# ctu-vras/depth_correction

Measured on AMD Instinct MI355X. Metric: points/sec through min_eigval_loss fwd+bwd (200k pts, k=10); HBM GB/s vs peak, higher is better.
Workload: dtype f64

## Files before the change

depth_correction_amd/csrc/dc_consistency.hip:

```cpp
#include <type_traits>
#include <atomic>
#include <mutex>
#include <cstdio>
#include <hip/hip_ext.h>
#include "dc_common.h"
#include "dc_device.h"
#include "dc_pointmath.h"
#include "dc_prof.h"
#include "dc_points_dev.h"
#include "../../include/dc_hip.h"

namespace dc {

template <typename T, typename PT, int STRIDE>
__global__ __launch_bounds__(kBlock) void points_fwd_kernel(PointInputs in, int64_t n, QParams qp, PT* __restrict__ x_out,
                                                            T* __restrict__ vps_out, T* __restrict__ dirs_out,
                                                            T* __restrict__ depth_out) {
  __shared__ double s_pose[kLdsScans * 12];
  const int64_t i = (int64_t)blockIdx.x * kBlock + threadIdx.x;
  const int64_t ic = i < n ? i : n - 1;
  ModelParams mp;
  load_model(in, mp);
  T vp_r[3] = {T(0), T(0), T(0)}, dr_r[3];
  if (in.vps) { const T* q = (const T*)in.vps + ic * 3; vp_r[0] = q[0]; vp_r[1] = q[1]; vp_r[2] = q[2]; }
// ... 1643 lines not shown
#pragma unroll
      for (int q = 1; q < NS; ++q) mx = max(mx, pre[q]);
      const bool any_miss = __any((int)(mx == kNoLoc)) != 0;
      int n_have;
      if (any_miss) n_have = gather_fixed<PT, NS, true>(tile, cap, ci, pre, acc);
      else n_have = gather_fixed<PT, NS, false>(tile, cap, ci, pre, acc);
      acc.W = (double)n_have;
      double cm[3], v0[3], c1, c2;
      if constexpr ((VAR & kVarSlimTail) != 0) step_point2<PT, NS>(acc, n_have, !any_miss, in_mask, lp, qp, acc2, cm, v0, &c1, &c2);
      else step_point<PT>(acc, in_mask, lp, qp, acc2, cm, v0, &c1, &c2);
      const double u = Pt<PT>::unit(qp);
      if constexpr ((VAR & kVarF32Sweep) != 0 && std::is_same<PT, q32>::value) {
        float cmf[3], vs[3], vu[3], gwf[P];
#pragma unroll
        for (int a = 0; a < 3; ++a) { cmf[a] = (float)cm[a]; vs[a] = (float)(c1 * v0[a]); vu[a] = (float)v0[a]; }
        const float c2f = (float)c2;
#pragma unroll
        for (int k = 0; k < P; ++k) gwf[k] = 0.0f;
        if (any_miss) {
#pragma unroll
          for (int q = 0; q < NS; ++q) {
            if (q % 4 == 0 && q > 0) __builtin_amdgcn_sched_barrier(0);
            chain_term_f32<P>(tile, cap, pre[q], pre[q] != kNoLoc, ci, cmf, vs, vu, c2f, gwf);
          }
        } else {
#pragma unroll
          for (int q = 0; q < NS; ++q) {
            if (q % 4 == 0 && q > 0) __builtin_amdgcn_sched_barrier(0);
            chain_term_f32<P>(tile, cap, pre[q], true, ci, cmf, vs, vu, c2f, gwf);
          }
        }
#pragma unroll
        for (int k = 0; k < P; ++k) gw[k] = (double)gwf[k] * u;
      } else {
        double mean[3];
        StepRow<PT, P>::mean_of(ci, cm, mean);
        if (any_miss) {
#pragma unroll
          for (int q = 0; q < NS; ++q) chain_term<PT, P>(tile, cap, pre[q], pre[q] != kNoLoc, mean, v0, c1, c2, gw);
        } else {
#pragma unroll
          for (int q = 0; q < NS; ++q) chain_term<PT, P>(tile, cap, pre[q], true, mean, v0, c1, c2, gw);
        }
#pragma unroll
        for (int k = 0; k < P; ++k) gw[k] *= u;
      }
    }
  }
  if (bad) acc2[0] = acc2[1] = __longlong_as_double(0x7ff8000000000000ll);
  step_partials<P, (VAR & kVarDppSums) != 0>(acc2, gw, p_fwd, p_bwd, chained, chained ? ch.n_front : 0);
}

constexpr int kStepQ32Cap = 512;

typedef float float2v __attribute__((ext_vector_type(2)));
template <int P, int CAP>
__device__ __forceinline__ void chain_term_q32(const int4* tile, uint32_t off, bool have, const Pt<q32>::Raw& ci, const float* cmf, const float* vs,
                                               const float* vu, float c2f, float* gw) {
  const char* row = reinterpret_cast<const char*>(tile) + (have ? off : 0u);
  const int4 p0 = *reinterpret_cast<const int4*>(row);
  const int4 p1 = *reinterpret_cast<const int4*>(row + (size_t)CAP * 16);
  const float2v e01 = float2v{(float)(p0.x - ci.v[0]), (float)(p0.y - ci.v[1])} - float2v{cmf[0], cmf[1]};
  const float e0 = e01.x, e1 = e01.y, e2 = (float)(p0.z - ci.v[2]) - cmf[2];
  const float u0 = __int_as_float(p0.w), u1 = __int_as_float(p1.x), u2 = __int_as_float(p1.y);
  const float al = fmaf(vs[2], e2, fmaf(vs[1], e1, vs[0] * e0));
  const float be = fmaf(vu[2], u2, fmaf(vu[1], u1, vu[0] * u0));
  const float ga = fmaf(e2, u2, fmaf(e1, u1, e0 * u0));
  float tj = fmaf(al, be, -(c2f * ga));
  if (!have) tj = 0.0f;
  if constexpr (P == 2) {
    float2v g = float2v{gw[0], gw[1]};
    g = __builtin_elementwise_fma(float2v{tj, tj}, float2v{__int_as_float(p1.z), __int_as_float(p1.w)}, g);
    gw[0] = g.x; gw[1] = g.y;
  } else {
    gw[0] = fmaf(tj, __int_as_float(p1.z), gw[0]);
    if constexpr (P > 1) gw[1] = fmaf(tj, __int_as_float(p1.w), gw[1]);
    if constexpr (P > 2) gw[2] = fmaf(tj, __int_as_float(reinterpret_cast<const int4*>(row + (size_t)CAP * 32)->x), gw[2]);
  }
}

#ifdef DC_BLOCK_TRACE
__device__ unsigned long long* g_block_trace = nullptr;
#define DC_TRACE_BEGIN() const unsigned long long trace_t0 = __builtin_amdgcn_s_memrealtime()
#define DC_TRACE_END() do { if (threadIdx.x == 0 && g_block_trace) { \
    unsigned long long* tr_ = g_block_trace + 4 * (size_t)blockIdx.x; \
    tr_[0] = ((unsigned long long)__builtin_amdgcn_s_getreg((31 << 11) | 20) << 32) | (unsigned)__builtin_amdgcn_s_getreg((31 << 11) | 4); \
    tr_[1] = trace_t0; tr_[2] = __builtin_amdgcn_s_memrealtime(); tr_[3] = 1; } } while (0)
#else
#define DC_TRACE_BEGIN() do {} while (0)
#define DC_TRACE_END() do {} while (0)
#endif

template <int NS, int P, int CAP>
__global__ __launch_bounds__(kBlock, (StepRow<q32, P>::kPieces * CAP * 16 <= 25 * 1024 ? 6 : 4)) void consistency_step_q32_kernel(
    PointBasis pb, BlockTab tab, const int32_t* __restrict__ own_base, const int32_t* __restrict__ centre_idx, int64_t n,
    const uint8_t* __restrict__ mask, LossParams lp, QParams qp, double* __restrict__ p_fwd, double* __restrict__ p_bwd,
    StepChain ch) {
  constexpr int NV = 2 + P, NP2 = NV <= 4 ? 4 : 8;
  constexpr int cap = CAP;
  __shared__ int4 tile[StepRow<q32, P>::kPieces * CAP];
  __shared__ double s_w[DC_MAX_MODEL_TERMS];
  __shared__ double s_front[kWavesPerBlock];
  __shared__ double s_comb[kWavesPerBlock * NP2];
  __shared__ int s_ok[2];
  DC_TRACE_BEGIN();
  const bool chained = ch.ready != nullptr;
  if (chained && (int)blockIdx.x < ch.n_front) { chain_front_block<P>(ch, s_front); return; }
  const int64_t nblocks = (n + kBlock - 1) / kBlock;
  int64_t blk = chain_block_of(ch, chained, nblocks);
  if (blk >= 0 && ch.blk_skip && ch.blk_skip[blk]) blk = -1;
  double acc2[2] = {0.0, 0.0}, gw[P];
#pragma unroll
  for (int k = 0; k < P; ++k) gw[k] = 0.0;
  const int32_t s0 = blk >= 0 ? tab.slot_ptr[blk] : 0;
  bool bad = blk >= 0 && tab.slot_ptr[blk + 1] - s0 != NS;
  if (blk >= 0 && !bad) {
    const int64_t i = blk * kBlock + threadIdx.x;
    const bool live = i < n;
    const bool in_mask = live && (mask ? mask[i] != 0 : true);
    const uint16_t* lrow = tab.loc + (int64_t)s0 * kBlock + threadIdx.x;
    uint32_t pre[NS];
#pragma unroll
    for (int q = 0; q < NS; ++q) pre[q] = (uint32_t)lrow[q * kBlock];
    const int32_t base = tab.blk_ptr[blk], nd = tab.blk_ptr[blk + 1] - base;
    const int32_t own = (own_base && !centre_idx) ? own_base[blk] : -1;
    double wq[P];
    if (chained) {
      typename StepRow<q32, P>::Raw r0, r1;
      const int t0 = threadIdx.x, t1 = threadIdx.x + kBlock;
      if (t0 < nd) r0 = StepRow<q32, P>::fetch(pb, tab.blk_ids[base + t0]);
      if (t1 < nd) r1 = StepRow<q32, P>::fetch(pb, tab.blk_ids[base + t1]);
      chain_weights<P>(ch, pb.w_scale, s_w, s_ok);
      __syncthreads();
      if (!s_ok[0]) bad = true;
#pragma unroll
      for (int k = 0; k < P; ++k) wq[k] = s_w[k];
      if (t0 < nd) StepRow<q32, P>::place(r0, wq, tile, cap, t0);
      if (t1 < nd) StepRow<q32, P>::place(r1, wq, tile, cap, t1);
      for (int t = threadIdx.x + 2 * kBlock; t < nd; t += kBlock) StepRow<q32, P>::stage(pb, wq, tab.blk_ids[base + t], tile, cap, t);
    } else {
      stage_weights(pb, s_w);
      __syncthreads();
#pragma unroll
      for (int k = 0; k < P; ++k) wq[k] = s_w[k];
      for (int t = threadIdx.x; t < nd; t += kBlock) StepRow<q32, P>::stage(pb, wq, tab.blk_ids[base + t], tile, cap, t);
    }
    Pt<q32>::Raw ci;
    if (own < 0) ci = Basis<q32>::template point<P>(pb, wq, live ? (centre_idx ? (int64_t)centre_idx[i] : i) : 0);
    __syncthreads();
    if (own >= 0) ci = staged_point<q32>(tile, cap, own + (live ? (int)threadIdx.x : 0));
    if (live && (!mask || __any((int)in_mask))) {
      CovAcc acc;
      cov_init(acc);
      uint32_t mo = pre[0];
#pragma unroll
      for (int q = 1; q < NS; ++q) mo |= pre[q];
      const bool any_miss = __any((int)(mo & 1u)) != 0;
      int n_have;
      if (any_miss) n_have = gather_fixed<q32, NS, true>(tile, cap, ci, pre, acc);
      else n_have = gather_fixed<q32, NS, false>(tile, cap, ci, pre, acc);
      acc.W = (double)n_have;
      double cm[3], v0[3], c1, c2;
      step_point2<q32, NS>(acc, n_have, !any_miss, in_mask, lp, qp, acc2, cm, v0, &c1, &c2);
      float cmf[3], vs[3], vu[3], gwf[P];
#pragma unroll
      for (int a = 0; a < 3; ++a) { cmf[a] = (float)cm[a]; vs[a] = (float)(c1 * v0[a]); vu[a] = (float)v0[a]; }
      const float c2f = (float)c2;
#pragma unroll
      for (int k = 0; k < P; ++k) gwf[k] = 0.0f;
      if (any_miss) {
#pragma unroll
        for (int q = 0; q < NS; ++q) {
          if (q % 4 == 0 && q > 0) __builtin_amdgcn_sched_barrier(0);
          chain_term_q32<P, CAP>(tile, pre[q], pre[q] != kNoLoc, ci, cmf, vs, vu, c2f, gwf);
        }
      } else {
#pragma unroll
        for (int q = 0; q < NS; ++q) {
          if (q % 4 == 0 && q > 0) __builtin_amdgcn_sched_barrier(0);
          chain_term_q32<P, CAP>(tile, pre[q], true, ci, cmf, vs, vu, c2f, gwf);
        }
      }
      const double u = qp.scale;
#pragma unroll
      for (int k = 0; k < P; ++k) gw[k] = (double)gwf[k] * u;
    }
  }
  if (bad) acc2[0] = acc2[1] = __longlong_as_double(0x7ff8000000000000ll);
  double v[NP2];
  v[0] = acc2[0]; v[1] = acc2[1];
#pragma unroll
  for (int k = 0; k < NP2 - 2; ++k) v[2 + k] = k < P ? gw[k] : 0.0;
  double tot;
  if constexpr (NP2 == 4) tot = wave_sum4_dpp(v);
  else tot = wave_sum_packed<NP2>(v);
  const int lane = threadIdx.x & (kWave - 1), wave = threadIdx.x / kWave;
  int64_t rs = (int64_t)gridDim.x * kWavesPerBlock, row = (int64_t)blockIdx.x * kWavesPerBlock + wave;
  if (chained) {
    if (lane < NP2) s_comb[wave * NP2 + lane] = tot;
    __syncthreads();
    if (wave != 0) return;
    if (lane < NP2) tot = (s_comb[lane] + s_comb[NP2 + lane]) + (s_comb[2 * NP2 + lane] + s_comb[3 * NP2 + lane]);
    rs = (int64_t)gridDim.x - ch.n_front;
    row = (int64_t)blockIdx.x - ch.n_front;
  }
  if (lane < NP2) {
    const int q = packed_value_of_lane<NP2>(lane);
    if (q < 2) p_fwd[q * rs + row] = tot;
    else if (q < NV) p_bwd[(q - 2) * rs + row] = tot;
  }
  DC_TRACE_END();
}

template <typename PT, int P>
__global__ __launch_bounds__(kBlock) void consistency_step_basis_slots_kernel(
    PointBasis pb, BlockTab tab, const int32_t* __restrict__ own_base, int cap, const int32_t* __restrict__ centre_idx, int64_t n,
    const uint8_t* __restrict__ mask, LossParams lp, QParams qp, double* __restrict__ p_fwd, double* __restrict__ p_bwd,
    StepChain ch, int packed) {
  extern __shared__ int4 tile[];
  __shared__ double s_w[DC_MAX_MODEL_TERMS];
  __shared__ int s_ok;
  __shared__ double s_front[kBlock / kWave];
  const bool chained = ch.ready != nullptr;
  if (chained && (int)blockIdx.x < ch.n_front) { chain_front_block<P>(ch, s_front); return; }
  const int64_t nblocks = (n + kBlock - 1) / kBlock;
  int64_t blk = xcd_block_of((int64_t)blockIdx.x - (chained ? ch.n_front : 0), nblocks);
  if (blk >= 0 && ch.blk_skip && ch.blk_skip[blk]) blk = -1;
  double acc2[2] = {0.0, 0.0}, gw[P];
#pragma unroll
  for (int k = 0; k < P; ++k) gw[k] = 0.0;
  const int64_t i = blk * kBlock + threadIdx.x;
  const bool live = blk >= 0 && i < n;
  int32_t nslots = 0, own = -1, base = 0, nd = 0;
  const uint16_t* lrow = tab.loc;
  uint32_t pre[kPreSlots];
  if (blk >= 0) {
    const int32_t s0 = tab.slot_ptr[blk];
    nslots = tab.slot_ptr[blk + 1] - s0;
    lrow = tab.loc + (int64_t)s0 * kBlock + threadIdx.x;
#pragma unroll
    for (int q = 0; q < kPreSlots; ++q) pre[q] = (live && q < nslots) ? (uint32_t)lrow[q * kBlock] : kNoLoc;
    own = (own_base && !centre_idx) ? own_base[blk] : -1;
    base = tab.blk_ptr[blk];
    nd = tab.blk_ptr[blk + 1] - base;
  }
  double wq[P];
  bool timed_out = false;
  typename Pt<PT>::Raw ci;
  if (chained) {
    typename StepRow<PT, P>::Raw r0, r1;
    const int t0 = threadIdx.x, t1 = threadIdx.x + kBlock;
    if (t0 < nd) r0 = StepRow<PT, P>::fetch(pb, tab.blk_ids[base + t0]);
    if (t1 < nd) r1 = StepRow<PT, P>::fetch(pb, tab.blk_ids[base + t1]);
    chain_weights<P>(ch, pb.w_scale, s_w, &s_ok);
    __syncthreads();
    timed_out = !s_ok;
#pragma unroll
    for (int k = 0; k < P; ++k) wq[k] = s_w[k];
    if (t0 < nd) StepRow<PT, P>::place(r0, wq, tile, cap, t0);
    if (t1 < nd) StepRow<PT, P>::place(r1, wq, tile, cap, t1);
    for (int t = threadIdx.x + 2 * kBlock; t < nd; t += kBlock) StepRow<PT, P>::stage(pb, wq, tab.blk_ids[base + t], tile, cap, t);
  } else {
    stage_weights(pb, s_w);
    __syncthreads();
#pragma unroll
    for (int k = 0; k < P; ++k) wq[k] = s_w[k];
    for (int t = threadIdx.x; t < nd; t += kBlock) StepRow<PT, P>::stage(pb, wq, tab.blk_ids[base + t], tile, cap, t);
  }
  if (blk >= 0 && own < 0) ci = Basis<PT>::template point<P>(pb, wq, live ? (centre_idx ? (int64_t)centre_idx[i] : i) : 0);
  __syncthreads();
  if (live) {
    if (own >= 0) ci = staged_point<PT>(tile, cap, own + (int)threadIdx.x);
    CovAcc acc;
    cov_init(acc);
    bool miss = false;
#pragma unroll
    for (int q = 0; q < kPreSlots; ++q) miss |= (q < nslots) && pre[q] == kNoLoc;
    int n_have = 0;
    if (__any((int)miss)) n_have = gather_slots<PT, true>(tile, cap, ci, pre, nslots, acc);
    else n_have = gather_slots<PT, false>(tile, cap, ci, pre, nslots, acc);
    if (nslots > kPreSlots) n_have += gather_tail<PT>(tile, cap, ci, lrow, nslots, packed != 0, acc);
    acc.W = (double)n_have;
    double cm[3], v0[3], c1, c2;
    step_point2<PT, 2>(acc, n_have, false, mask ? mask[i] != 0 : true, lp, qp, acc2, cm, v0, &c1, &c2);
    const double u = Pt<PT>::unit(qp);
    if constexpr (std::is_same<PT, q32>::value) {
      float cmf[3], vs[3], vu[3], gwf[P];
#pragma unroll
      for (int a = 0; a < 3; ++a) { cmf[a] = (float)cm[a]; vs[a] = (float)(c1 * v0[a]); vu[a] = (float)v0[a]; }
      const float c2f = (float)c2;
#pragma unroll
      for (int k = 0; k < P; ++k) gwf[k] = 0.0f;
#pragma unroll
      for (int q = 0; q < kPreSlots; ++q)
// ... 89 lines not shown
    cov_init(acc);
    auto sweep1 = [&](const uint32_t* l, uint32_t* nx, const uint16_t* pn) {
#pragma unroll
      for (int u_ = 0; u_ < kTrip; ++u_) nx[u_] = (uint32_t)pn[u_ * kBlock];
      int4 r[kTrip];
#pragma unroll
      for (int u_ = 0; u_ < kTrip; ++u_) r[u_] = *reinterpret_cast<const int4*>(tb + (l[u_] == kNoLoc ? own_off : l[u_]));
#pragma unroll
      for (int u_ = 0; u_ < kTrip; ++u_)
        cov_add_d(acc, (double)(r[u_].x - ci.v[0]), (double)(r[u_].y - ci.v[1]), (double)(r[u_].z - ci.v[2]));
    };
    {
      uint32_t la[kTrip], lb[kTrip];
#pragma unroll
      for (int u_ = 0; u_ < kTrip; ++u_) la[u_] = first[u_];
      const uint16_t* pn = lrow + kTrip * kBlock;
      for (int q0 = 0; q0 < wmax; q0 += 2 * kTrip) {
        sweep1(la, lb, pn);
        pn += kTrip * kBlock;
        if (q0 + kTrip >= wmax) break;
        sweep1(lb, la, pn);
        pn += kTrip * kBlock;
      }
    }
    acc.W = (double)deg;
    double cm[3], v0[3], c1, c2;
    step_point2<q32, 2>(acc, deg, false, in_mask, lp, qp, acc2, cm, v0, &c1, &c2);
    const double u = Pt<q32>::unit(qp);
    float cmf[3], vs[3], vu[3];
#pragma unroll
    for (int a = 0; a < 3; ++a) { cmf[a] = (float)cm[a]; vs[a] = (float)(c1 * v0[a]); vu[a] = (float)v0[a]; }
    const float c2f = (float)c2;
    auto sweep2 = [&](const uint32_t* l, uint32_t* nx, const uint16_t* pn) {
#pragma unroll
      for (int u_ = 0; u_ < kTrip; ++u_) nx[u_] = (uint32_t)pn[u_ * kBlock];
      float2v g[P];
#pragma unroll
      for (int k = 0; k < P; ++k) g[k] = float2v{0.0f, 0.0f};
#pragma unroll
      for (int u_ = 0; u_ < kTrip; u_ += 2) {
        const bool ha = l[u_] != kNoLoc, hb = l[u_ + 1] != kNoLoc;
        const char* ra = tb + (ha ? l[u_] : own_off);
        const char* rb = tb + (hb ? l[u_ + 1] : own_off);
        const int4 a0 = *reinterpret_cast<const int4*>(ra), a1 = *reinterpret_cast<const int4*>(ra + CAP * 16);
        const int4 b0 = *reinterpret_cast<const int4*>(rb), b1 = *reinterpret_cast<const int4*>(rb + CAP * 16);
        const float2v e0 = float2v{(float)(a0.x - ci.v[0]), (float)(b0.x - ci.v[0])} - float2v{cmf[0], cmf[0]};
        const float2v e1 = float2v{(float)(a0.y - ci.v[1]), (float)(b0.y - ci.v[1])} - float2v{cmf[1], cmf[1]};
        const float2v e2 = float2v{(float)(a0.z - ci.v[2]), (float)(b0.z - ci.v[2])} - float2v{cmf[2], cmf[2]};
        const float2v u0 = float2v{__int_as_float(a0.w), __int_as_float(b0.w)};
        const float2v u1 = float2v{__int_as_float(a1.x), __int_as_float(b1.x)};
        const float2v u2 = float2v{__int_as_float(a1.y), __int_as_float(b1.y)};
        const float2v al = __builtin_elementwise_fma(float2v{vs[2], vs[2]}, e2, __builtin_elementwise_fma(float2v{vs[1], vs[1]}, e1, float2v{vs[0], vs[0]} * e0));
        const float2v be = __builtin_elementwise_fma(float2v{vu[2], vu[2]}, u2, __builtin_elementwise_fma(float2v{vu[1], vu[1]}, u1, float2v{vu[0], vu[0]} * u0));
        const float2v ga = __builtin_elementwise_fma(e2, u2, __builtin_elementwise_fma(e1, u1, e0 * u0));
        float2v tj = __builtin_elementwise_fma(al, be, -(float2v{c2f, c2f} * ga));
        tj = float2v{ha ? tj.x : 0.0f, hb ? tj.y : 0.0f};
        g[0] = __builtin_elementwise_fma(tj, float2v{__int_as_float(a1.z), __int_as_float(b1.z)}, g[0]);
        if constexpr (P > 1) g[1] = __builtin_elementwise_fma(tj, float2v{__int_as_float(a1.w), __int_as_float(b1.w)}, g[1]);
        if constexpr (P > 2)
          g[2] = __builtin_elementwise_fma(tj, float2v{__int_as_float(reinterpret_cast<const int4*>(ra + CAP * 32)->x),
                                                       __int_as_float(reinterpret_cast<const int4*>(rb + CAP * 32)->x)}, g[2]);
      }
#pragma unroll
      for (int k = 0; k < P; ++k) gw[k] += (double)(g[k].x + g[k].y);
    };
    {
      uint32_t la[kTrip], lb[kTrip];
#pragma unroll
      for (int u_ = 0; u_ < kTrip; ++u_) la[u_] = first[u_];
      const uint16_t* pn = lrow + kTrip * kBlock;
      for (int q0 = 0; q0 < wmax; q0 += 2 * kTrip) {
        sweep2(la, lb, pn);
        pn += kTrip * kBlock;
        if (q0 + kTrip >= wmax) break;
        sweep2(lb, la, pn);
        pn += kTrip * kBlock;
      }
    }
#pragma unroll
    for (int k = 0; k < P; ++k) gw[k] *= u;
  }
  if (timed_out) acc2[0] = acc2[1] = __longlong_as_double(0x7ff8000000000000ll);
  step_partials<P, true>(acc2, gw, p_fwd, p_bwd, chained, chained ? ch.n_front : 0);
  DC_TRACE_END();
}

struct PoseTab {
  const int32_t* __restrict__ blk_ptr;
  const int32_t* __restrict__ ids;
  const uint16_t* __restrict__ loc;
  const uint16_t* __restrict__ own_pos;
  const uint16_t* __restrict__ row_seg;
  const uint8_t* __restrict__ row_scan;
};
constexpr int kPoseCap = 512;

template <int K>
__global__ __launch_bounds__(kBlock) void pose_table_kernel(BlockTab tab, const int32_t* __restrict__ own_base,
                                                            const int32_t* __restrict__ scan_id, int64_t n, int n_scans,
                                                            int32_t* __restrict__ ids_out, uint16_t* __restrict__ loc_out,
                                                            uint16_t* __restrict__ own_pos, uint16_t* __restrict__ row_seg,
                                                            uint8_t* __restrict__ row_scan, int32_t* __restrict__ info) {
  __shared__ int32_t s_id[kPoseCap];
  __shared__ uint8_t s_scan[kPoseCap];
  __shared__ uint16_t s_new[kPoseCap];
  __shared__ int s_start[kMaxBlockScans + 1];
  const int64_t b = blockIdx.x;
  const int tid = threadIdx.x;
  const int32_t base = tab.blk_ptr[b], nd = tab.blk_ptr[b + 1] - base;
  const int32_t own = own_base[b];
  if (nd > kPoseCap || own < 0 || tab.slot_ptr[b + 1] - tab.slot_ptr[b] != K) {
    if (tid == 0) atomicMax(info, 1);
    return;
  }
  if (tid <= n_scans) s_start[tid] = 0;
  __syncthreads();
  for (int t = tid; t < nd; t += kBlock) {
    const int32_t id = tab.blk_ids[base + t];
    const int sc = scan_id ? scan_id[id] : 0;
    s_id[t] = id;
    s_scan[t] = (uint8_t)sc;
    atomicAdd(&s_start[sc + 1], 1);
  }
  __syncthreads();
  if (tid == 0) for (int q = 0; q < n_scans; ++q) s_start[q + 1] += s_start[q];
  __syncthreads();
  for (int t = tid; t < nd; t += kBlock) {
    const int sc = s_scan[t];
    int rank = 0;
    for (int t2 = 0; t2 < t; ++t2) rank += s_scan[t2] == sc ? 1 : 0;
    const int p = s_start[sc] + rank;
    s_new[t] = (uint16_t)p;
    ids_out[base + p] = s_id[t];
    row_scan[base + p] = (uint8_t)sc;
  }
  if (tid <= n_scans) row_seg[b * (n_scans + 1) + tid] = (uint16_t)s_start[tid];
  __syncthreads();
  const int64_t i = b * kBlock + tid;
  if (i < n) own_pos[i] = (uint16_t)(s_new[own + tid] << 4);
  const uint16_t* lrow = tab.loc + (int64_t)tab.slot_ptr[b] * kBlock + tid;
#pragma unroll
  for (int q = 0; q < K; ++q) {
    const uint16_t l = lrow[q * kBlock];
    loc_out[((int64_t)b * K + q) * kBlock + tid] = l == 0xFFFF ? (uint16_t)0xFFFF : (uint16_t)(s_new[l >> 4] << 4);
  }
}

template <typename T>
__global__ __launch_bounds__(kBlock) void points_local_basis_kernel(PointInputs in, PoseTab tab, int32_t* __restrict__ rows) {
  const int64_t b = blockIdx.x;
  const int32_t base = tab.blk_ptr[b], nd = tab.blk_ptr[b + 1] - base;
  ModelParams mp;
  load_model(in, mp);
  for (int t = threadIdx.x; t < nd; t += kBlock) {
    const int64_t i = tab.ids[base + t];
    const T* dp = (const T*)in.dirs + i * 3;
    const double d = (double)((const T*)in.depth)[i];
    const bool lm = in.lmask ? in.lmask[i] != 0 : true;
    const bool on = mp.kind != DC_MODEL_NONE && lm;
    const double inc = on ? (double)((const T*)in.inc)[i] : 0.0;
    const double d0 = (on && mp.kind == DC_MODEL_LINEAR) ? 0.0 : d;
    float c[2] = {0.0f, 0.0f};
#pragma unroll
    for (int k = 0; k < 2; ++k) {
      if (k < mp.n_terms && on) {
        const double dk = mp.kind > DC_MODEL_SCALED_POLYNOMIAL ? model_dw_other(mp, k, d, inc)
                                                               : (mp.kind == DC_MODEL_SCALED_POLYNOMIAL ? -d : -1.0) * pow_term(inc, mp.e[k]);
// ... 375 lines not shown
  }
}

__global__ __launch_bounds__(kRedBlock) void reduce_eval_kernel(const double* __restrict__ p_fwd, const double* __restrict__ p_bwd,
                                                                int64_t rows_fwd, int64_t rows_bwd, int n_red, int n_out,
                                                                double* __restrict__ out, AdamArgs adam,
                                                                const int32_t* __restrict__ status, int pose_first = -1,
                                                                int pose_cols = 0) {
  __shared__ double lds[kRedBlock / kWave * kPoseRedCols];
  const int a = blockIdx.x;
  if (a == 0)
    for (int z = 2 + n_red + threadIdx.x; z < n_out; z += kRedBlock) out[z] = 0.0;
  const int lane = threadIdx.x & (kWave - 1), wave = threadIdx.x / kWave;
  if (pose_first >= 0 && a >= 2 + pose_first) {
    const int col = (a - 2 - pose_first) * kPoseRedCols + (threadIdx.x & (kPoseRedCols - 1));
    const bool have = col < pose_cols;
    const double* p = p_bwd + (int64_t)pose_first * rows_bwd + (have ? col : 0);
    double s = strided_sum(p, have ? rows_bwd / kWavesPerBlock : 0, pose_cols, threadIdx.x / kPoseRedCols, kRedBlock / kPoseRedCols);
#pragma unroll
    for (int o = kPoseRedCols; o < kWave; o <<= 1) s += __shfl_xor(s, o, kWave);
    if (lane < kPoseRedCols) lds[wave * kPoseRedCols + lane] = s;
    __syncthreads();
    if (threadIdx.x < kPoseRedCols && have) {
      double t = 0.0;
      for (int wv = 0; wv < kRedBlock / kWave; ++wv) t += lds[wv * kPoseRedCols + threadIdx.x];
      out[2 + pose_first + col] = t;
    }
    return;
  }
  const bool flagged = a == 0 && threadIdx.x == 0 && status && *status != 0;
  const int64_t n_rows = a < 2 ? rows_fwd : rows_bwd;
  const double* p = a < 2 ? p_fwd + (int64_t)a * rows_fwd : p_bwd + (int64_t)(a - 2) * rows_bwd;
  const bool step = adam.p && a >= 2 && a - 2 < adam.n && threadIdx.x == 0;
  double p0 = 0.0, m0 = 0.0, v0 = 0.0;
  if (step) { p0 = adam.p[a - 2]; m0 = adam.m[a - 2]; v0 = adam.v[a - 2]; }
  const double s = wave_sum(strided_sum(p, n_rows));
  if (lane == 0) lds[wave] = s;
  __syncthreads();
  if (threadIdx.x == 0) {
    double t = 0.0;
    for (int wv = 0; wv < kRedBlock / kWave; ++wv) t += lds[wv];
    if (flagged) t = __longlong_as_double(0x7ff8000000000000ll);
    out[a] = t;
    if (step) adam_apply(adam, a - 2, t, p0, m0, v0);
  }
}

static inline unsigned red_grid(int n_red, int pose_first, int pose_cols) {
  if (pose_first < 0 || n_red <= pose_first) return 2u + (unsigned)n_red;
  return 2u + (unsigned)pose_first + (unsigned)((pose_cols + kPoseRedCols - 1) / kPoseRedCols);
}

__global__ void adam_kernel(const double* __restrict__ grad, AdamArgs adam) {
  const int i = (int)(blockIdx.x * blockDim.x + threadIdx.x);
  if (i < adam.n) adam_update(adam, i, grad[i]);
}

__global__ __launch_bounds__(256) void adam_device_step_kernel(const double* __restrict__ grad, AdamArgs adam, int64_t* __restrict__ step) {
  const double t = (double)(*step + 1);
  adam.bias1 = 1.0 - pow(adam.b1, t);
  adam.bias2_sqrt = sqrt(1.0 - pow(adam.b2, t));
  for (int i = threadIdx.x; i < adam.n; i += blockDim.x) adam_update(adam, i, grad[i]);
  __syncthreads();
  if (threadIdx.x == 0) *step = (int64_t)t;
}

}

using namespace dc;

#define DC_CHECK_LAUNCH()                                  \
  do {                                                     \
    hipError_t err__ = hipGetLastError();                  \
    if (err__ != hipSuccess) return (int)err__;            \
  } while (0)

static inline int64_t n_blocks(int64_t n) { return (n + kBlock - 1) / kBlock; }
static std::atomic<bool> g_no_reverse{false};
static std::atomic<bool> g_pose_three_pass{false};
static std::atomic<bool> g_no_tab{false};
static std::atomic<int> g_fwd_generic{0};
static std::atomic<bool> g_two_pass{false};
static std::atomic<int> g_step_var{1};
static std::atomic<int> g_chain_spin{1 << 22};
static std::atomic<bool> g_no_basis{false};

template <int P, int CAP>
static int ragged_launch(dim3 grid, hipStream_t stream, hipEvent_t ev0, hipEvent_t ev1, const PointBasis& pb, const BlockTab& tab,
                         const dcBlockTable* t, int64_t n_rows, const uint8_t* mask, const LossParams& lp, const QParams& qp, double* p_fwd,
                         double* p_bwd, const StepChain& ch) {
  constexpr size_t bytes = (size_t)StepRow<q32, P>::kPieces * CAP * 16;
  static std::atomic<uint64_t> attr_set{0};
  if (bytes > 60 * 1024) {
    int dev = 0;
    if (hipGetDevice(&dev) != hipSuccess) dev = 0;
    const uint64_t bit = 1ull << (dev & 63);
    if (!(attr_set.fetch_or(bit) & bit)) {
      hipError_t err = hipFuncSetAttribute((const void*)consistency_step_ragged_q32_kernel<P, CAP>, hipFuncAttributeMaxDynamicSharedMemorySize, (int)bytes);
      if (err != hipSuccess) { attr_set.fetch_and(~bit); return (int)err; }
    }
  }
  hipExtLaunchKernelGGL((consistency_step_ragged_q32_kernel<P, CAP>), grid, dim3(kBlock), bytes, stream, ev0, ev1, 0, pb, tab, t->own_base, t->row_ptr, n_rows,
                        mask, lp, qp, p_fwd, p_bwd, ch);
  return DC_OK;
}

static bool use_table(const dcBlockTable* t, int layout, int stride, uint32_t row_bytes, int extra_rows, size_t lds_limit,
                      size_t* lds_bytes, int* lds_rows) {
  if (!t || g_no_tab.load() || stride != 4 || t->layout != layout || !t->blk_ptr || !t->loc || t->max_rows < 0) return false;
  if (layout == DC_TABLE_SLOTS ? !t->slot_ptr : !t->run_ptr) return false;
  if (t->max_rows > 0 && !t->blk_ids) return false;
  const size_t rows = (size_t)t->max_rows + extra_rows + (t->max_rows + extra_rows == 0 ? 1 : 0);
  const size_t need = rows * row_bytes;
  if (need > lds_limit || t->max_rows >= 0xFFF) return false;
  *lds_bytes = need;
  *lds_rows = (int)rows;
  return true;
}

extern "C" {

int dc_version(void) { return 100; }

int64_t dc_partial_rows(int64_t n) { return xcd_grid(n_blocks(n)) * kWavesPerBlock; }

int dc_param_grad_count(int n_terms, int n_scans) { return 2 * n_terms + 12 * n_scans; }

int64_t dc_sequence_partials_count(int64_t n, int n_terms, int n_scans) {
  if (n < 0 || n_terms < 0 || n_scans < 0) return 0;
  const int64_t rows = xcd_grid(n_blocks(n)) * kWavesPerBlock;
  return rows * (2 + 2 * (int64_t)n_terms + 12 * (int64_t)n_scans) + 2 * (2 + (int64_t)n_terms) * rows;
}

static PointInputs make_inputs(const void* vps, const void* dirs, const void* depth, const void* inc,
                               const uint8_t* lmask, const int32_t* scan_id, const double* poses, int n_scans,
                               int model_kind, int n_terms, const double* w, const double* e) {
  PointInputs in;
  in.vps = vps; in.dirs = dirs; in.depth = depth; in.inc = inc; in.lmask = lmask; in.scan_id = scan_id;
  in.poses = poses; in.w = w; in.e = e; in.model_kind = model_kind; in.n_terms = n_terms; in.n_scans = n_scans;
  return in;
}

static int check_model(int model_kind, int n_terms, const void* inc, const double* w, const double* e) {
  if (model_kind < DC_MODEL_NONE || model_kind > DC_MODEL_LAST) return DC_ERR_ARG;
  if (model_kind != DC_MODEL_NONE) {
    if (n_terms < 1 || n_terms > DC_MAX_MODEL_TERMS || !inc || !w || !e) return DC_ERR_ARG;
    if (model_kind == DC_MODEL_LINEAR && n_terms != 3) return DC_ERR_ARG;
    if ((model_kind == DC_MODEL_INVCOS || model_kind == DC_MODEL_SCALED_INVCOS) && n_terms != 1) return DC_ERR_ARG;
  }
  return DC_OK;
}

static int make_qparams(int point_fmt, int dtype, int stride, const double* qparams, QParams* qp, int32_t* flag = nullptr) {
  *qp = QParams{};
  qp->flag = flag;
  if (point_fmt == DC_Q32) {
    if (!qparams || stride != 4 || dtype != DC_F32 || !(qparams[3] > 0.0)) return DC_ERR_ARG;
    qp->origin[0] = qparams[0]; qp->origin[1] = qparams[1]; qp->origin[2] = qparams[2];
    qp->scale = qparams[3];
    qp->inv_scale = 1.0 / qparams[3];
    return DC_OK;
  }
  return point_fmt == dtype ? DC_OK : DC_ERR_DTYPE;
}

#define DC_DISPATCH_FMT(dtype, fmt, stride, LAUNCH)                       \
// ... 406 lines not shown
}

static int sequence_eval_impl(const dcSequenceDesc* d, const double* w, const double* e, const double* poses, int want_grad,
                              int want_exponent_grad, int want_pose_grad, double* out, hipStream_t stream,
                              const AdamArgs& adam, const ChainCall* chain = nullptr, bool one_pass_only = false) {
  if (!d || !out || !poses || !d->partials) return DC_ERR_ARG;
  if (!one_pass_only && d->fwd_table_loss && d->mask && !d->centre_idx && want_grad && !want_exponent_grad && !want_pose_grad && d->basis &&
      d->model_kind != DC_MODEL_NONE && d->n_terms >= 1 && d->n_terms <= 3 && d->n > 0) {
    dcSequenceDesc dd = *d;
    dd.fwd_table = d->fwd_table_loss;
    dd.fwd_table_loss = nullptr;
    dd.fwd_rows_active = d->fwd_rows_active_loss;
    const int rc = sequence_eval_impl(&dd, w, e, poses, want_grad, want_exponent_grad, want_pose_grad, out, stream, adam, chain, true);
    if (rc != DC_ERR_UNSUPPORTED) return rc;
  }
  const int stride = 4;
  const int n_terms = d->model_kind == DC_MODEL_NONE ? 0 : d->n_terms;
  const int n_acc = 2 * n_terms + 12 * d->n_scans;
  if (d->n == 0) return (int)hipMemsetAsync(out, 0, (size_t)(2 + n_acc) * sizeof(double), stream);
  if (d->partials_count < dc_sequence_partials_count(d->n, n_terms, d->n_scans)) return DC_ERR_WORKSPACE;
  const int64_t n_rows = d->centre_idx ? d->n_centres : d->n;
  if (d->centre_idx && (d->n_centres < 0 || d->n_centres > d->n)) return DC_ERR_ARG;
  const int64_t rows = xcd_grid(n_blocks(d->n)) * kWavesPerBlock;
  double* p_fwd = d->partials;
  double* p_bwd = d->partials + 2 * rows;
  const int n_red = !want_grad ? 0 : (want_pose_grad ? n_acc : 2 * n_terms);

  size_t lds_f = 0, lds_b = 0;
  int rows_f = 0, rows_b = 0;
  const bool q32_pts = d->point_fmt == DC_Q32 && d->dtype == DC_F32, f64_pts = d->point_fmt == DC_F64 && d->dtype == DC_F64;
  const int rag_pieces = n_terms <= 2 ? 2 : 3;
  const int rag_rows = !d->fwd_table ? 0 : ((d->blk_skip && d->mask && !d->centre_idx && d->fwd_rows_active > 0 && d->fwd_rows_active < d->fwd_table->max_rows)
                                              ? d->fwd_rows_active : d->fwd_table->max_rows);
  const bool ragged_ok = q32_pts && d->fwd_table && d->fwd_table->layout == DC_TABLE_SLOTS && d->fwd_table->packed == 1 && d->fwd_table->row_ptr &&
                         d->fwd_table->own_base && !d->centre_idx && d->fwd_table->max_rows > 0 && !g_no_tab.load() && g_step_var.load() != 8 &&
                         (size_t)rag_rows * rag_pieces * 16 <= 128 * 1024 && rag_rows <= (n_terms <= 2 ? 4096 : 2560);
  const bool basis_fwd = d->basis && (q32_pts || f64_pts) && n_terms > 0 && w &&
                         !want_exponent_grad && !want_pose_grad && !g_no_basis.load() &&
                         (use_table(d->fwd_table, DC_TABLE_SLOTS, stride, q32_pts ? 16u : 32u, 0, 60 * 1024, &lds_f, &rows_f) || (ragged_ok && want_grad && n_terms <= 3 && !g_two_pass.load()));
  size_t lds_s = 0;
  int rows_s = 0;
  const unsigned step_row_bytes = 16u * (unsigned)(q32_pts ? (6 + n_terms + 3) / 4 : 3);
  dcBlockTable ft_active{};
  if (d->fwd_table) {
    ft_active = *d->fwd_table;
    if (d->blk_skip && d->mask && !d->centre_idx && d->fwd_rows_active > 0 && d->fwd_rows_active < ft_active.max_rows) ft_active.max_rows = d->fwd_rows_active;
  }
  const bool one_pass = basis_fwd && want_grad && n_terms <= 3 && !g_two_pass.load() &&
                        (use_table(d->fwd_table ? &ft_active : nullptr, DC_TABLE_SLOTS, stride, step_row_bytes, 0, 60 * 1024, &lds_s, &rows_s) || ragged_ok);
  const bool pose_one_pass = want_grad && want_pose_grad && !want_exponent_grad && d->pose_table && d->local_basis && !d->vps && !d->centre_idx &&
                             d->point_fmt == DC_Q32 && d->dtype == DC_F32 && (n_terms == 1 || n_terms == 2) && d->n_scans <= kLdsScans && w &&
                             (d->k == 4 || d->k == 8 || d->k == 10 || d->k == 16) && !g_pose_three_pass.load();
  if (want_grad && !one_pass && !pose_one_pass && (!d->csr_ptr || !d->csr_src)) return DC_ERR_BACKWARD_TABLES;
  const bool basis = basis_fwd &&
                     (!want_grad || one_pass || use_table(d->bwd_table, DC_TABLE_RUNS, stride, q32_pts ? 32u : 64u, 1, 44 * 1024, &lds_b, &rows_b));
  const int fixed_k = g_fwd_generic.load() ? 0 : d->k;
  if ((chain || one_pass_only) && !(basis && one_pass)) return DC_ERR_UNSUPPORTED;
  if (basis) {
    QParams qp;
    int rc = make_qparams(d->point_fmt, d->dtype, stride, d->qparams, &qp);
    if (rc) return rc;
    PointBasis pb{d->basis, w, n_terms, q32_pts ? qp.inv_scale : 1.0};
    const LossParams lp = make_loss_params(d->loss_kind & ~DC_LOSS_RAW_POINTWISE, d->normalization, d->sqrt_);
    BlockTab tab{d->fwd_table->blk_ptr, d->fwd_table->blk_ids, d->fwd_table->slot_ptr, d->fwd_table->loc};
    const dim3 block(kBlock);
    if (one_pass) {
      const int64_t g_blocks = xcd_grid(n_blocks(n_rows));
      StepChain ch{};
      ch.blk_skip = (d->mask && !d->centre_idx) ? d->blk_skip : nullptr;
      if (chain) {
        p_fwd = chain_buffer(d, n_terms, chain->parity);
        p_bwd = p_fwd + 2 * g_blocks;
        ch.ready = chain->ready; ch.parity = chain->parity; ch.has_prev = chain->has_prev; ch.n_front = kChainFront;
        ch.n_out = 2 + n_acc; ch.prev = chain_buffer(d, n_terms, chain->parity ^ 1); ch.prev_rows = g_blocks;
        if (chain->prev_rows) { ch.prev = chain->prev_rows; ch.prev_rows = chain->prev_count; }
        ch.acc_in = chain->acc_in; ch.prev_status = chain->prev_status;
        ch.out_prev = chain->out_prev; ch.w_prev_out = chain->w_prev_out; ch.status = d->status; ch.spin_limit = g_chain_spin.load(); ch.adam = chain->adam_prev;
        ch.grad_sum = chain->grad_sum;
        ch.stamp = chain->stamp; ch.w_now = w;
        ch.reverse = (chain->parity && !g_no_reverse.load()) ? 1 : 0;
      }
      const dim3 grid((unsigned)(g_blocks + (chain ? kChainFront : 0)));
      const int var = g_step_var.load();
      const bool q32_step = q32_pts && var == 1 && (fixed_k == 10 || fixed_k == 4 || fixed_k == 8 || fixed_k == 16) && rows_s <= 768;
      const bool ragged_step = ragged_ok;
      if (ragged_step) {
        ProfScope prof(1);
        const int mr = rag_rows;
        int rc = DC_OK;
#define RAGGED(P, CAP) (prof.name("(consistency_step_ragged_q32_kernel<" #P ", " #CAP ">)"), \
                        ragged_launch<P, CAP>(grid, stream, prof.start(), prof.stop(), pb, tab, d->fwd_table, n_rows, d->mask, lp, qp, p_fwd, p_bwd, ch))
#define RAGGED_CAPS(P) (mr <= 1024 ? RAGGED(P, 1024) : mr <= 1280 ? RAGGED(P, 1280) : mr <= 1600 ? RAGGED(P, 1600) : mr <= 2048 ? RAGGED(P, 2048) : \
                        mr <= 2560 ? RAGGED(P, 2560) : RAGGED(P, 4096))
        if (n_terms == 2) rc = RAGGED_CAPS(2);
        else if (n_terms == 1) rc = RAGGED_CAPS(1);
        else rc = mr <= 1024 ? RAGGED(3, 1024) : mr <= 1600 ? RAGGED(3, 1600) : RAGGED(3, 2560);
#undef RAGGED_CAPS
#undef RAGGED
        if (rc) return rc;
      } else if (q32_step) {
        ProfScope prof(1);
        static_assert(kStepQ32Cap == 512, "the profiler names the instantiation by its literal arguments");
#define STEPQ_LAUNCH(NS, P, CAP) DC_TIMED_LAUNCH((consistency_step_q32_kernel<NS, P, CAP>), grid, block, 0, stream, pb, tab, d->fwd_table->own_base, \
                                                 d->centre_idx, n_rows, d->mask, lp, qp, p_fwd, p_bwd, ch)
#define STEPQ_P(NS, CAP) do { if (n_terms == 2) STEPQ_LAUNCH(NS, 2, CAP); else if (n_terms == 1) STEPQ_LAUNCH(NS, 1, CAP); else STEPQ_LAUNCH(NS, 3, CAP); } while (0)
#define STEPQ_K(CAP) do { if (fixed_k == 10) STEPQ_P(10, CAP); else if (fixed_k == 4) STEPQ_P(4, CAP); else if (fixed_k == 8) STEPQ_P(8, CAP); else STEPQ_P(16, CAP); } while (0)
        if (rows_s <= 512) STEPQ_K(512); else STEPQ_K(768);
#undef STEPQ_K
#undef STEPQ_P
#undef STEPQ_LAUNCH
      } else {
        ProfScope prof(1);
#define STEP_LAUNCH(K) DC_TIMED_LAUNCH(K, grid, block, lds_s, stream, pb, tab, d->fwd_table->own_base, rows_s, d->centre_idx, n_rows, \
                                       d->mask, lp, qp, p_fwd, p_bwd, ch)
#define STEP_NS(PT, P) do { if (fixed_k == 10 && P == 2 && var == 0) STEP_LAUNCH((consistency_step_basis_kernel<PT, 10, 2, 0>)); \
                            else if (fixed_k == 10) STEP_LAUNCH((consistency_step_basis_kernel<PT, 10, P, kStepVar>)); \
                            else if (fixed_k == 4) STEP_LAUNCH((consistency_step_basis_kernel<PT, 4, P, kStepVar>)); \
                            else if (fixed_k == 8) STEP_LAUNCH((consistency_step_basis_kernel<PT, 8, P, kStepVar>)); \
                            else if (fixed_k == 16) STEP_LAUNCH((consistency_step_basis_kernel<PT, 16, P, kStepVar>)); \
                            else DC_TIMED_LAUNCH((consistency_step_basis_slots_kernel<PT, P>), grid, block, lds_s, stream, pb, tab, d->fwd_table->own_base, rows_s, \
                                                 d->centre_idx, n_rows, d->mask, lp, qp, p_fwd, p_bwd, ch, d->fwd_table->packed); } while (0)
#define STEP(PT) do { if (n_terms == 2) STEP_NS(PT, 2); else if (n_terms == 1) STEP_NS(PT, 1); else STEP_NS(PT, 3); } while (0)
        if (q32_pts) STEP(q32); else STEP(double);
#undef STEP
#undef STEP_NS
#undef STEP_LAUNCH
      }
      DC_CHECK_LAUNCH();
      if (chain && chain->reduce_now) {
        hipLaunchKernelGGL(reduce_eval_kernel, dim3(2 + n_terms), dim3(kRedBlock), 0, stream, p_fwd, p_bwd, g_blocks, g_blocks, n_terms,
                           2 + n_acc, out, AdamArgs{}, (const int32_t*)d->status);
        DC_CHECK_LAUNCH();
      }
      if (chain) return DC_OK;
      const int64_t rows_g = (int64_t)grid.x * kWavesPerBlock;
      hipLaunchKernelGGL(reduce_eval_kernel, dim3(2 + n_terms), dim3(kRedBlock), 0, stream, p_fwd, p_bwd, rows_g, rows_g, n_terms, 2 + n_acc, out,
                         adam, (const int32_t*)d->status);
      DC_CHECK_LAUNCH();
      return DC_OK;
    }
    {
      ProfScope prof(1);
      const dim3 grid((unsigned)xcd_grid(n_blocks(n_rows)));
#define FWD_BASIS_P(PT, T, NS, P) DC_TIMED_LAUNCH((consistency_fwd_basis_kernel<PT, false, NS, P>), grid, block, lds_f, stream, pb, tab, \
                                                 d->fwd_table->own_base, rows_f, d->centre_idx, n_rows, d->mask, (const T*)nullptr, lp, qp, \
                                                 (PT*)(want_grad ? d->rec : nullptr), (T*)nullptr, (T*)nullptr, p_fwd)
#define FWD_BASIS_SLOTS(PT, T, P) DC_TIMED_LAUNCH((consistency_fwd_basis_slots_kernel<PT, false, P>), grid, block, lds_f, stream, pb, tab, \
                                                 d->fwd_table->own_base, rows_f, d->centre_idx, n_rows, d->mask, (const T*)nullptr, lp, qp, \
                                                 (PT*)(want_grad ? d->rec : nullptr), (T*)nullptr, (T*)nullptr, p_fwd)
#define FWD_BASIS_NS(PT, T, P) do { if (fixed_k == 10) FWD_BASIS_P(PT, T, 10, P); else if (fixed_k == 4) FWD_BASIS_P(PT, T, 4, P); \
                                    else if (fixed_k == 8) FWD_BASIS_P(PT, T, 8, P); else if (fixed_k == 16) FWD_BASIS_P(PT, T, 16, P); \
                                    else FWD_BASIS_SLOTS(PT, T, P); } while (0)
#define FWD_BASIS(PT, T) do { if (n_terms == 2) FWD_BASIS_NS(PT, T, 2); else if (n_terms == 1) FWD_BASIS_NS(PT, T, 1); \
                              else if (n_terms == 3) FWD_BASIS_NS(PT, T, 3); else FWD_BASIS_NS(PT, T, 0); } while (0)
      if (q32_pts) FWD_BASIS(q32, float); else FWD_BASIS(double, double);
#undef FWD_BASIS
#undef FWD_BASIS_NS
#undef FWD_BASIS_SLOTS
#undef FWD_BASIS_P
    }
    DC_CHECK_LAUNCH();
    if (want_grad) {
      RunTab rtab{d->bwd_table->blk_ptr, d->bwd_table->blk_ids, d->bwd_table->run_ptr, d->bwd_table->loc};
      ProfScope prof(2);
#define BWD_BASIS_P(PT, P) DC_TIMED_LAUNCH((consistency_bwd_basis_kernel<PT, P>), dim3((unsigned)xcd_grid(n_blocks(d->n))), block, lds_b, stream, pb, \
                                          (const PT*)d->rec, rtab, rows_b, d->n, qp, p_bwd)
#define BWD_BASIS(PT) do { if (n_terms == 2) BWD_BASIS_P(PT, 2); else if (n_terms == 1) BWD_BASIS_P(PT, 1); \
                           else if (n_terms == 3) BWD_BASIS_P(PT, 3); else BWD_BASIS_P(PT, 0); } while (0)
      if (q32_pts) BWD_BASIS(q32); else BWD_BASIS(double);
#undef BWD_BASIS
#undef BWD_BASIS_P
      DC_CHECK_LAUNCH();
    }
    hipLaunchKernelGGL(reduce_eval_kernel, dim3(2 + n_red), dim3(kRedBlock), 0, stream, p_fwd, p_bwd,
                       xcd_grid(n_blocks(n_rows)) * kWavesPerBlock, rows, n_red, 2 + n_acc, out, adam, (const int32_t*)d->status);
    DC_CHECK_LAUNCH();
    return DC_OK;
  }

  if (pose_one_pass) {
    QParams qp;
    int rc = make_qparams(d->point_fmt, d->dtype, stride, d->qparams, &qp, d->status);
    if (rc) return rc;
    const dcPoseTable* pt = d->pose_table;
    PoseTab tab{pt->blk_ptr, pt->ids, pt->loc, pt->own_pos, pt->row_seg, pt->row_scan};
    const LossParams lp = make_loss_params(d->loss_kind & ~DC_LOSS_RAW_POINTWISE, d->normalization, d->sqrt_);
    const dim3 grid((unsigned)xcd_grid(n_blocks(d->n))), block(kBlock);
    {
      ProfScope prof(1);
#define POSE_NS(NS, P) DC_TIMED_LAUNCH((consistency_step_pose_kernel<NS, P>), grid, block, 0, stream, (const int32_t*)d->local_basis, tab, poses, d->n_scans, \
                                       w, d->n, d->mask, lp, qp, p_fwd, p_bwd)
#define POSE_P(NS) do { if (n_terms == 2) POSE_NS(NS, 2); else POSE_NS(NS, 1); } while (0)
      if (d->k == 10) POSE_P(10); else if (d->k == 4) POSE_P(4); else if (d->k == 8) POSE_P(8); else POSE_P(16);
// ... 184 lines not shown
```

Before: 51.69 billion.

## Let idle waves exit early and reduce block partials through LDS in q32 step

The q32 consistency step kernel now records, per wave, whether it has any live or masked-in points. Waves with no work return right after staging instead of running the gather and reduction. Partial sums of the remaining waves are handed to the first running wave through the reused tile LDS, so each block writes a single partial row instead of one per wave, padding the other slots with zeros. The old per-wave form stays behind a variant flag. This adds extra barriers and LDS traffic in the reduction, and it changes the layout of the partial-sum buffer.

```diff
diff --git a/depth_correction_amd/csrc/dc_consistency.hip b/depth_correction_amd/csrc/dc_consistency.hip
--- a/depth_correction_amd/csrc/dc_consistency.hip
+++ b/depth_correction_amd/csrc/dc_consistency.hip
@@ -1749,27 +1749,61 @@
 #ifdef DC_BLOCK_TRACE
 __device__ unsigned long long* g_block_trace = nullptr;
 #define DC_TRACE_BEGIN() const unsigned long long trace_t0 = __builtin_amdgcn_s_memrealtime()
-#define DC_TRACE_END() do { if (threadIdx.x == 0 && g_block_trace) { \
+#define DC_TRACE_END(first) do { if ((first) && g_block_trace) { \
     unsigned long long* tr_ = g_block_trace + 4 * (size_t)blockIdx.x; \
     tr_[0] = ((unsigned long long)__builtin_amdgcn_s_getreg((31 << 11) | 20) << 32) | (unsigned)__builtin_amdgcn_s_getreg((31 << 11) | 4); \
     tr_[1] = trace_t0; tr_[2] = __builtin_amdgcn_s_memrealtime(); tr_[3] = 1; } } while (0)
 #else
 #define DC_TRACE_BEGIN() do {} while (0)
-#define DC_TRACE_END() do {} while (0)
+#define DC_TRACE_END(first) do {} while (0)
 #endif
 
-template <int NS, int P, int CAP>
+constexpr int kStepWaveSums = 0, kStepEarlyExit = 1;
+
+template <int P>
+__device__ __forceinline__ bool block_sums(const double* acc2, const double* gw, int runs, int wave, double* hand, double* tot) {
+  constexpr int NV = 2 + P, NP2 = NV <= 4 ? 4 : 8;
+  double v[NP2];
+  v[0] = acc2[0]; v[1] = acc2[1];
+#pragma unroll
+  for (int k = 0; k < NP2 - 2; ++k) v[2 + k] = k < P ? gw[k] : 0.0;
+  const int first = __builtin_ctz(runs);
+  if (runs & (runs - 1)) {
+    __syncthreads();
+    if (wave != first) {
+#pragma unroll
+      for (int c = 0; c < NV; ++c) hand[c * kBlock + threadIdx.x] = v[c];
+    }
+    __syncthreads();
+    if (wave != first) return false;
+    const int lane = threadIdx.x & (kWave - 1);
+#pragma unroll
+    for (int w = 1; w < kWavesPerBlock; ++w) {
+      if (w > first && ((runs >> w) & 1)) {
+#pragma unroll
+        for (int c = 0; c < NV; ++c) v[c] += hand[c * kBlock + w * kWave + lane];
+      }
+    }
+  }
+  if constexpr (NP2 == 4) *tot = wave_sum4_dpp(v);
+  else *tot = wave_sum_packed<NP2>(v);
+  return true;
+}
+
+template <int NS, int P, int CAP, int FORM = kStepEarlyExit>
 __global__ __launch_bounds__(kBlock, (StepRow<q32, P>::kPieces * CAP * 16 <= 25 * 1024 ? 6 : 4)) void consistency_step_q32_kernel(
     PointBasis pb, BlockTab tab, const int32_t* __restrict__ own_base, const int32_t* __restrict__ centre_idx, int64_t n,
     const uint8_t* __restrict__ mask, LossParams lp, QParams qp, double* __restrict__ p_fwd, double* __restrict__ p_bwd,
     StepChain ch) {
   constexpr int NV = 2 + P, NP2 = NV <= 4 ? 4 : 8;
   constexpr int cap = CAP;
+  static_assert(NV * kBlock * sizeof(double) <= StepRow<q32, P>::kPieces * CAP * sizeof(int4), "block_sums hands over through the tile");
   __shared__ int4 tile[StepRow<q32, P>::kPieces * CAP];
   __shared__ double s_w[DC_MAX_MODEL_TERMS];
   __shared__ double s_front[kWavesPerBlock];
-  __shared__ double s_comb[kWavesPerBlock * NP2];
+  __shared__ double s_comb[FORM == kStepWaveSums ? kWavesPerBlock * NP2 : 1];
   __shared__ int s_ok[2];
+  __shared__ uint32_t s_kinds;
   DC_TRACE_BEGIN();
   const bool chained = ch.ready != nullptr;
   if (chained && (int)blockIdx.x < ch.n_front) { chain_front_block<P>(ch, s_front); return; }
@@ -1781,10 +1815,18 @@
   for (int k = 0; k < P; ++k) gw[k] = 0.0;
   const int32_t s0 = blk >= 0 ? tab.slot_ptr[blk] : 0;
   bool bad = blk >= 0 && tab.slot_ptr[blk + 1] - s0 != NS;
+  const int lane = threadIdx.x & (kWave - 1), wave = __builtin_amdgcn_readfirstlane((int)threadIdx.x / kWave);
+  int runs = 0;
+  const auto leave = [&](bool run) {
+    const uint32_t k = __builtin_amdgcn_readfirstlane(s_kinds);
+    runs = (int)((k & 1u) | ((k >> 7) & 2u) | ((k >> 14) & 4u) | ((k >> 21) & 8u));
+    return !run && wave != (runs ? __builtin_ctz(runs) : 0);
+  };
   if (blk >= 0 && !bad) {
     const int64_t i = blk * kBlock + threadIdx.x;
     const bool live = i < n;
     const bool in_mask = live && (mask ? mask[i] != 0 : true);
+    const auto wave_runs = [&] { return (mask ? __any((int)in_mask) : __any((int)live)) != 0; };
     const uint16_t* lrow = tab.loc + (int64_t)s0 * kBlock + threadIdx.x;
     uint32_t pre[NS];
 #pragma unroll
@@ -1814,9 +1856,16 @@
     }
     Pt<q32>::Raw ci;
     if (own < 0) ci = Basis<q32>::template point<P>(pb, wq, live ? (centre_idx ? (int64_t)centre_idx[i] : i) : 0);
+    const bool run = wave_runs();
+    if constexpr (FORM == kStepEarlyExit) {
+      if (lane == 0) reinterpret_cast<uint8_t*>(&s_kinds)[wave] = run ? 1 : 0;
+    }
     __syncthreads();
+    if constexpr (FORM == kStepEarlyExit) {
+      if (leave(run)) return;
+    }
     if (own >= 0) ci = staged_point<q32>(tile, cap, own + (live ? (int)threadIdx.x : 0));
-    if (live && (!mask || __any((int)in_mask))) {
+    if (run && live) {
       CovAcc acc;
       cov_init(acc);
       uint32_t mo = pre[0];
@@ -1852,31 +1901,48 @@
 #pragma unroll
       for (int k = 0; k < P; ++k) gw[k] = (double)gwf[k] * u;
     }
+  } else {
+    if constexpr (FORM != kStepWaveSums) {
+      if (wave != 0) return;
+    }
   }
   if (bad) acc2[0] = acc2[1] = __longlong_as_double(0x7ff8000000000000ll);
-  double v[NP2];
-  v[0] = acc2[0]; v[1] = acc2[1];
-#pragma unroll
-  for (int k = 0; k < NP2 - 2; ++k) v[2 + k] = k < P ? gw[k] : 0.0;
   double tot;
-  if constexpr (NP2 == 4) tot = wave_sum4_dpp(v);
-  else tot = wave_sum_packed<NP2>(v);
-  const int lane = threadIdx.x & (kWave - 1), wave = threadIdx.x / kWave;
-  int64_t rs = (int64_t)gridDim.x * kWavesPerBlock, row = (int64_t)blockIdx.x * kWavesPerBlock + wave;
+  int64_t rs = (int64_t)gridDim.x * kWavesPerBlock, row = (int64_t)blockIdx.x * kWavesPerBlock;
+  if constexpr (FORM == kStepWaveSums) {
+    double v[NP2];
+    v[0] = acc2[0]; v[1] = acc2[1];
+#pragma unroll
+    for (int k = 0; k < NP2 - 2; ++k) v[2 + k] = k < P ? gw[k] : 0.0;
+    if constexpr (NP2 == 4) tot = wave_sum4_dpp(v);
+    else tot = wave_sum_packed<NP2>(v);
+    row += wave;
+    if (chained) {
+      if (lane < NP2) s_comb[wave * NP2 + lane] = tot;
+      __syncthreads();
+      if (wave != 0) return;
+      if (lane < NP2) tot = (s_comb[lane] + s_comb[NP2 + lane]) + (s_comb[2 * NP2 + lane] + s_comb[3 * NP2 + lane]);
+    }
+  } else {
+    if (runs) {
+      if (!block_sums<P>(acc2, gw, runs, wave, reinterpret_cast<double*>(tile), &tot)) return;
+    } else {
+      tot = (bad && packed_value_of_lane<NP2>(lane) < 2) ? __longlong_as_double(0x7ff8000000000000ll) : 0.0;
+    }
+  }
   if (chained) {
-    if (lane < NP2) s_comb[wave * NP2 + lane] = tot;
-    __syncthreads();
-    if (wave != 0) return;
-    if (lane < NP2) tot = (s_comb[lane] + s_comb[NP2 + lane]) + (s_comb[2 * NP2 + lane] + s_comb[3 * NP2 + lane]);
     rs = (int64_t)gridDim.x - ch.n_front;
     row = (int64_t)blockIdx.x - ch.n_front;
   }
   if (lane < NP2) {
     const int q = packed_value_of_lane<NP2>(lane);
-    if (q < 2) p_fwd[q * rs + row] = tot;
-    else if (q < NV) p_bwd[(q - 2) * rs + row] = tot;
-  }
-  DC_TRACE_END();
+    if (q < NV) {
+      double* col = (q < 2 ? p_fwd + q * rs : p_bwd + (q - 2) * rs) + row;
+      col[0] = tot;
+      if (FORM != kStepWaveSums && !chained) { col[1] = 0.0; col[2] = 0.0; col[3] = 0.0; }
+    }
+  }
+  DC_TRACE_END(FORM == kStepWaveSums ? threadIdx.x == 0 : lane == 0);
 }
 
 template <typename PT, int P>
@@ -2132,7 +2198,7 @@
   }
   if (timed_out) acc2[0] = acc2[1] = __longlong_as_double(0x7ff8000000000000ll);
   step_partials<P, true>(acc2, gw, p_fwd, p_bwd, chained, chained ? ch.n_front : 0);
-  DC_TRACE_END();
+  DC_TRACE_END(threadIdx.x == 0);
 }
 
 struct PoseTab {
@@ -2674,6 +2740,7 @@
 static std::atomic<int> g_fwd_generic{0};
 static std::atomic<bool> g_two_pass{false};
 static std::atomic<int> g_step_var{1};
+constexpr int kVarWaveSums = 16;
 static std::atomic<int> g_chain_spin{1 << 22};
 static std::atomic<bool> g_no_basis{false};
 
@@ -3246,7 +3313,7 @@
       }
       const dim3 grid((unsigned)(g_blocks + (chain ? kChainFront : 0)));
       const int var = g_step_var.load();
-      const bool q32_step = q32_pts && var == 1 && (fixed_k == 10 || fixed_k == 4 || fixed_k == 8 || fixed_k == 16) && rows_s <= 768;
+      const bool q32_step = q32_pts && (var & ~kVarWaveSums) == 1 && (fixed_k == 10 || fixed_k == 4 || fixed_k == 8 || fixed_k == 16) && rows_s <= 768;
       const bool ragged_step = ragged_ok;
       if (ragged_step) {
         ProfScope prof(1);
@@ -3265,14 +3332,19 @@
       } else if (q32_step) {
         ProfScope prof(1);
         static_assert(kStepQ32Cap == 512, "the profiler names the instantiation by its literal arguments");
-#define STEPQ_LAUNCH(NS, P, CAP) DC_TIMED_LAUNCH((consistency_step_q32_kernel<NS, P, CAP>), grid, block, 0, stream, pb, tab, d->fwd_table->own_base, \
-                                                 d->centre_idx, n_rows, d->mask, lp, qp, p_fwd, p_bwd, ch)
+#define STEPQ_FORM(NS, P, CAP, FORM) DC_TIMED_LAUNCH((consistency_step_q32_kernel<NS, P, CAP, FORM>), grid, block, 0, stream, pb, tab, \
+                                                     d->fwd_table->own_base, d->centre_idx, n_rows, d->mask, lp, qp, p_fwd, p_bwd, ch)
+#define STEPQ_LAUNCH(NS, P, CAP) STEPQ_FORM(NS, P, CAP, kStepEarlyExit)
 #define STEPQ_P(NS, CAP) do { if (n_terms == 2) STEPQ_LAUNCH(NS, 2, CAP); else if (n_terms == 1) STEPQ_LAUNCH(NS, 1, CAP); else STEPQ_LAUNCH(NS, 3, CAP); } while (0)
 #define STEPQ_K(CAP) do { if (fixed_k == 10) STEPQ_P(10, CAP); else if (fixed_k == 4) STEPQ_P(4, CAP); else if (fixed_k == 8) STEPQ_P(8, CAP); else STEPQ_P(16, CAP); } while (0)
-        if (rows_s <= 512) STEPQ_K(512); else STEPQ_K(768);
+        const bool ab_shape = fixed_k == 10 && n_terms == 2 && rows_s <= 512;
+        if (ab_shape && (var & kVarWaveSums)) STEPQ_FORM(10, 2, 512, kStepWaveSums);
+        else if (rows_s <= 512) STEPQ_K(512);
+        else STEPQ_K(768);
 #undef STEPQ_K
 #undef STEPQ_P
 #undef STEPQ_LAUNCH
+#undef STEPQ_FORM
       } else {
         ProfScope prof(1);
 #define STEP_LAUNCH(K) DC_TIMED_LAUNCH(K, grid, block, lds_s, stream, pb, tab, d->fwd_table->own_base, rows_s, d->centre_idx, n_rows, \
```

New measurement: 51.65 billion (median of 3 runs). Within noise of the previous version (-0.1%).
